# mousecpn/Boosting-R-CNN

Measured on AMD Instinct MI355X. Metric: images/sec (1333x800) Boosting R-CNN R50-PAFPN inference, higher is better.
Workload: dtype f32; 1 GPU; boosting_rcnn_r50_pafpn_1x_utdac.py inference (model(return_loss=False, rescale=True): device pass + result copy + bbox2result), batch 8 x 3x800x1344 per GPU, f32 MFMA conv stack, 1000 pre-NMS / 256 proposals per image, seeded synthetic weights; global_batch=8, parallelism=dp1

## Files before the change

### boosting-r-cnn_amd/csrc/misc.hip

```cpp
#include "common.h"

namespace {

__device__ __forceinline__ float4 ld4(const float* p) { return *reinterpret_cast<const float4*>(p); }
__device__ __forceinline__ void st4(float* p, float4 v) { *reinterpret_cast<float4*>(p) = v; }
__device__ __forceinline__ float4 ld4(const bf16_t* p) {
    const uint2 u = *reinterpret_cast<const uint2*>(p);
    return make_float4(__uint_as_float(u.x << 16), __uint_as_float(u.x & 0xffff0000u),
                       __uint_as_float(u.y << 16), __uint_as_float(u.y & 0xffff0000u));
}
__device__ __forceinline__ unsigned f2bf(float v) { return brcnn_f2b(v); }
__device__ __forceinline__ void st4(bf16_t* p, float4 v) {
    uint2 u;
    u.x = brcnn_pk2b(v.x, v.y);
    u.y = brcnn_pk2b(v.z, v.w);
    *reinterpret_cast<uint2*>(p) = u;
}
__device__ __forceinline__ float4 ld4(const f16_t* p) {
    const uint2 u = *reinterpret_cast<const uint2*>(p);
    return make_float4(brcnn_h2f((unsigned short)(u.x & 0xffffu)), brcnn_h2f((unsigned short)(u.x >> 16)),
                       brcnn_h2f((unsigned short)(u.y & 0xffffu)), brcnn_h2f((unsigned short)(u.y >> 16)));
}
__device__ __forceinline__ void st4(f16_t* p, float4 v) {
    uint2 u;
// ... 895 lines not shown
    } else {
        if (int st = gn_forward_16<f16_t>(x, gamma, beta, y, stats_ws, sg, batch, num_segments, channels, groups, eps,
                                          relu, chunks, rpb, total, nstat, s))
            return st;
    }
    BRCNN_LAUNCH_CHECK();
    return 0;
}


static int gn_setup(GnSegs& sg, long long& rows, int& max_hw, int batch, int num_segments, const int* hw_host) {
    sg = GnSegs{};
    sg.nseg = num_segments;
    rows = 0;
    max_hw = 0;
    for (int i = 0; i < num_segments; i++) {
        if (hw_host[i] <= 0) return BRCNN_EINVAL;
        sg.hw[i] = hw_host[i];
        sg.row0[i] = rows;
        rows += (long long)batch * hw_host[i];
        if (hw_host[i] > max_hw) max_hw = hw_host[i];
    }
    for (int i = num_segments; i <= BRCNN_MAX_LEVELS; i++) sg.row0[i] = rows;
    return 0;
}

static void gn_bwd_chunks(int max_hw, int* chunks, int* rpb) {
    int c = (max_hw + 255) / 256;
    if (c > 64) c = 64;
    *rpb = (max_hw + c - 1) / c;
    *chunks = (max_hw + *rpb - 1) / *rpb;
}

BRCNN_API size_t brcnn_groupnorm_nhwc_multi_backward_workspace_bytes(int batch, int num_segments, const int* hw_host,
                                                                    int channels, int groups) {
    if (batch <= 0 || num_segments <= 0 || num_segments > BRCNN_MAX_LEVELS || !hw_host || channels <= 0 || groups <= 0)
        return 0;
    int max_hw = 0;
    for (int i = 0; i < num_segments; i++) max_hw = hw_host[i] > max_hw ? hw_host[i] : max_hw;
    int chunks, rpb;
    gn_bwd_chunks(max_hw, &chunks, &rpb);
    return (size_t)batch * num_segments * groups * 2 * sizeof(double) +
           ((size_t)batch * num_segments * chunks + GN_PARAM_SLICES) * 2 * channels * sizeof(float);
}

BRCNN_API int brcnn_groupnorm_nhwc_multi_backward(const void* dy, const void* x, const void* stats,
// ... 238 lines not shown
```

### boosting-r-cnn_amd/csrc/policy.h

```cpp
#pragma once

namespace brcnn {

struct Policy {
    int use_dma = 1;
    int force_wm = 0, force_nt = 0;
    int no_fast = 0;
    int pp_f32_n128 = 1;
    int pp_f32_mode = 1;
    int f32_tile_sk = 1;
    int f32_tile_sk_per_cu = 0;

    int bf16_tile = 0;
    int bf16_il = 0;
    int sk_mode = 1;
    int sk_par = 0;
    int pp_mode = 1;
    int pp128_mode = 1;
    int pp128_min_k = 4096;
    int pp128_max_t88 = 128;
    int sk_spin_limit = 1 << 24;
    int sk_drop_publish = 0;
    int stream_mode = 1;

    int wgrad_bf16_tile = 0;
    int wgrad_slabs = 1;
    int wgrad_slot_pct = 75;
    int wgrad_slot_pct_big = 75;
    int wgrad_two_pass = 24;
    int wgrad_pp_mode = 1;
    int wgrad_pp_slot_pct = 75;
    int wgrad_pp_two_pass = 24;
    int wgrad_pp_fuse = 0;

// ... 6 lines not shown
};
extern Policy g_policy;

struct Counters {
    int f32_tile_sk_launches = 0;
    int f32_tile_sk_wgs = 0;
    int wgrad_pp_launches = 0;
    int pp_f32_launches = 0;
    int pp_f32_rows = 0;
    int pp_f32_cols = 0;
    int pp_bf16_launches = 0;
    int pp128_bf16_launches = 0;
    int stream1x1_launches = 0;
    int sk_chain_fills = 0;
    int sk_par_fills = 0;
    int sk_last_wgs = 0;
    int bf16_tile_launches = 0;
    int bf16_tile_rows = 0;
    int bf16_tile_cols = 0;
    int bf16_tile_waves = 0;
    int bf16_tile_stages = 0;
    int wgrad_bf16_tile_launches = 0;
    int wgrad_bf16_last_tile = 0;
    int roi_ordered_launches = 0;
    int roi_prepared_launches = 0;
    int roi_gather_chunked = 0;
    int roi_gather_last_ch = 0;
};
extern Counters g_counters;
inline void count(int& c) { c = (c + 1) & 0x7fffffff; }

}
```

### boosting-r-cnn_amd/csrc/policy.hip

```cpp
#include "common.h"
#include "policy.h"

__attribute__((require_constant_initialization)) brcnn::Policy brcnn::g_policy;
__attribute__((require_constant_initialization)) brcnn::Counters brcnn::g_counters;
using brcnn::g_counters, brcnn::g_policy;

BRCNN_API int brcnn_conv_set_tile(int wm, int nt) {
    if (wm == -1) { g_policy.use_dma = nt; return 0; }
    if (wm == -3) { if (nt < 0 || nt > 2) return BRCNN_EINVAL; g_policy.pp_f32_n128 = nt; return 0; }
    if (wm == -4) { if (nt != 0 && nt != 1) return BRCNN_EINVAL; g_policy.no_fast = nt; return 0; }
    if (wm == -5) { if (nt < 0 || nt > 2) return BRCNN_EINVAL; g_policy.f32_tile_sk = nt; return 0; }
    if (wm == -7) { if (nt < 0 || nt > 8) return BRCNN_EINVAL; g_policy.f32_tile_sk_per_cu = nt; return 0; }
    if (wm == -6) return nt == 0 ? g_counters.f32_tile_sk_launches : nt == 1 ? g_counters.f32_tile_sk_wgs : BRCNN_EINVAL;
    if (wm == -9) {
        int* const c[] = {&g_counters.pp_f32_launches, &g_counters.pp_f32_rows, &g_counters.pp_f32_cols, &g_counters.pp_bf16_launches,
                          &g_counters.pp128_bf16_launches, &g_counters.stream1x1_launches, &g_counters.sk_chain_fills,
                          &g_counters.sk_par_fills, &g_counters.sk_last_wgs, &g_counters.bf16_tile_launches, &g_counters.bf16_tile_rows,
                          &g_counters.bf16_tile_cols, &g_counters.bf16_tile_waves, &g_counters.bf16_tile_stages,
                          &g_counters.wgrad_bf16_tile_launches, &g_counters.wgrad_bf16_last_tile};
        const int count = (int)(sizeof(c) / sizeof(c[0]));
        if (nt < -1 || nt >= count) return BRCNN_EINVAL;
        if (nt == -1) { for (int* q : c) *q = 0; return 0; }
        const int n = *c[nt];
        *c[nt] = 0;
        return n;
    }
    if (wm == -2) { if (nt != 0 && nt != 1 && nt != 2 && nt != 128 && nt != 256) return BRCNN_EINVAL; g_policy.pp_f32_mode = nt; return 0; }
    if ((wm != 0 && wm != 1 && wm != 2 && wm != 4) || nt < 0 || nt > 2) return BRCNN_EINVAL;
    g_policy.force_wm = wm;
    g_policy.force_nt = nt;
    return 0;
}

BRCNN_API int brcnn_conv_set_tile_bf16(int mtnt) {
    if (mtnt == -1 || mtnt == -2) { g_policy.bf16_il = (mtnt == -1); return 0; }
    if (mtnt <= -3 && mtnt >= -5) { g_policy.sk_mode = -3 - mtnt; return 0; }
    if (mtnt <= -8 && mtnt >= -10) { g_policy.sk_par = -8 - mtnt; return 0; }
    if (mtnt == -6 || mtnt == -7) { g_policy.pp_mode = mtnt == -7; return 0; }
    if (mtnt == -18 || mtnt == -19) { g_policy.pp128_mode = mtnt == -19; return 0; }
    if (mtnt <= -1000 && mtnt > -2000) { g_policy.pp128_min_k = -1000 - mtnt; return 0; }
    if (mtnt <= -2000 && mtnt > -3000) { g_policy.pp128_max_t88 = -2000 - mtnt; return 0; }
    if (mtnt <= -15 && mtnt >= -17) { g_policy.stream_mode = -15 - mtnt; return 0; }
    if (mtnt == -11 || mtnt == -12) { g_policy.sk_drop_publish = mtnt == -11; g_policy.sk_spin_limit = mtnt == -11 ? 256 : 1 << 24; return 0; }
    const int ok[] = {0, 11, 21, 22, 42, 82, 81, 164, 342, 382, 3164, 322, 482, 381, 2244, 2144, 8844, 8842};
    bool found = false;
    for (int v : ok) found |= (v == mtnt);
    if (!found) return BRCNN_EINVAL;
// ... 84 lines not shown
```

### boosting-r-cnn_amd/dense_heads.py

```python
import copy

import torch
import torch.distributed as dist
import torch.nn as nn

from . import ops
from .blocks import (ConvModule, PackedCache, Scale, bias_init_with_prob, pack_weight, to_nhwc)
from .postprocess import batched_nms_images
from .core import (anchor_inside_flags, bbox_overlaps, images_to_levels, multi_apply, unmap)
from .registry import (HEADS, build_anchor_generator, build_assigner, build_bbox_coder,
                       build_loss, build_sampler)

EPS = 1e-12


def cat_rows(feats):
    from .autograd import cat_rows as _cr
    return _cr(list(feats))


def reduce_mean(tensor):
    if not (dist.is_available() and dist.is_initialized()):
        return tensor
    tensor = tensor.clone()
# ... 91 lines not shown
                sampling_result)


@HEADS.register_module()
class ATSSRPNHead(AnchorHead):
    def __init__(self, in_channels, num_classes=1, stacked_convs=4, conv_cfg=None, gamma=1,
                 atss=False, bridge=False, last_conv='norm', aug_reg_loss=None,
                 norm_cfg=dict(type='GN', num_groups=32, requires_grad=True),
                 loss_centerness=dict(type='CrossEntropyLoss', use_sigmoid=True, loss_weight=0.5),
                 init_cfg=None, num_convs=1, **kwargs):
        assert not atss, 'atss=True (ATSSAssigner targets) is outside the shipped boosting configs'
        assert not bridge and last_conv == 'norm', 'bridge / dcn / aspp variants are out of scope'
        self.stacked_convs, self.conv_cfg, self.norm_cfg = stacked_convs, conv_cfg, norm_cfg
        self.last_conv = last_conv
        super().__init__(num_classes, in_channels, init_cfg=init_cfg, **kwargs)
        self.loss_centerness = build_loss(loss_centerness)
        self.gamma, self.atss, self.bridge = gamma, atss, bridge
        self.with_aug_loss = aug_reg_loss is not None
        if self.with_aug_loss:
            self.aug_loss = build_loss(aug_reg_loss)
        self._head_caches = [PackedCache() for _ in range(8)]
        self._tower_caches = [PackedCache() for _ in range(stacked_convs)]
        self._fused_head_cache = PackedCache()
        self._base_anchor_cache = {}
        self.init_weights()

    def _init_layers(self):
        self.rpn_convs = nn.ModuleList()
        for i in range(self.stacked_convs):
            chn = self.in_channels if i == 0 else self.feat_channels
            self.rpn_convs.append(ConvModule(chn, self.feat_channels, 3, stride=1, padding=1,
                                             conv_cfg=self.conv_cfg, norm_cfg=self.norm_cfg))
        self.rpn_cls = nn.Conv2d(self.feat_channels, self.num_anchors * self.cls_out_channels, 3,
                                 padding=1)
        self.rpn_reg = nn.Conv2d(self.feat_channels, self.num_anchors * 4, 3, padding=1)
        self.rpn_iou = nn.Conv2d(self.feat_channels, self.num_anchors * 1, 3, padding=1)
        self.scales = nn.ModuleList([Scale(1.0) for _ in self.anchor_generator.strides])

    def init_weights(self):
        for m in self.modules():
            if isinstance(m, nn.Conv2d):
                nn.init.normal_(m.weight, 0, 0.01)
                if m.bias is not None:
                    nn.init.constant_(m.bias, 0)
        nn.init.constant_(self.rpn_cls.bias, bias_init_with_prob(0.01))

# ... 50 lines not shown
        for conv in self.rpn_convs:
            x = conv2d_nhwc_multi_autograd(x, conv.conv.weight, None, B, sizes, 1, conv.conv.padding[0])
            x = GroupNormNHWCFunction.apply(x, conv.norm.weight, conv.norm.bias, conv.norm.num_groups, B, sizes,
                                            conv.norm.eps, conv.with_activation)
        heads = (self.rpn_cls, self.rpn_reg, self.rpn_iou)
        y = conv2d_nhwc_multi_autograd(x, torch.cat([h.weight for h in heads], 0),
                                       torch.cat([h.bias for h in heads], 0), B, sizes, 1,
                                       self.rpn_cls.padding[0], out_f32=True).float()
        a, c = self.num_anchors, self.cls_out_channels
        cls, reg, iou, r0 = [], [], [], 0
        for lvl, (h, w) in enumerate(sizes):
            n = B * h * w
            t = y[r0:r0 + n].view(B, h, w, y.shape[1])
            cls.append(t[..., :a * c])
            reg.append(t[..., a * c:a * c + 4 * a] * self.scales[lvl].scale)
            iou.append(t[..., a * c + 4 * a:])
            r0 += n
        return cls, reg, iou

    def forward_fused(self, feats):
        B = feats[0].shape[0]
        sizes = [tuple(f.shape[1:3]) for f in feats]
        x = cat_rows(feats)
        for i, conv in enumerate(self.rpn_convs):
            assert isinstance(conv.norm, nn.GroupNorm) and conv.conv.bias is None
            w = self._tower_caches[i].get([conv.conv.weight],
                                          lambda c=conv: pack_weight(c.conv.weight).to(x.dtype))
            x, _ = ops.conv2d_nhwc_multi(x, w, B, sizes, None, None, None, False, 1, 1)
            x = ops.groupnorm_nhwc_multi(x, conv.norm.weight.detach(), conv.norm.bias.detach(),
                                         conv.norm.num_groups, B, sizes, conv.norm.eps,
                                         conv.with_activation)
        heads = (self.rpn_cls, self.rpn_reg, self.rpn_iou)

        def builder():
            return (torch.cat([pack_weight(h.weight) for h in heads], 0).to(x.dtype).contiguous(),
                    torch.cat([h.bias.detach().float() for h in heads], 0).contiguous())
        w, b = self._fused_head_cache.get([t for h in heads for t in (h.weight, h.bias)], builder)
        y, _ = ops.conv2d_nhwc_multi(x, w, B, sizes, None, b, None, False, 1, 1, out_f32=True)
        outs, r0 = [], 0
        for (h, wd) in sizes:
            n = B * h * wd
            outs.append(y[r0:r0 + n].view(B, h, wd, y.shape[1]))
            r0 += n
        return outs

    def split_fused(self, fused):
        a, c = self.num_anchors, self.cls_out_channels
        cls = [f[..., :a * c] for f in fused]
        reg = [f[..., a * c:a * c + 4 * a] for f in fused]
        iou = [f[..., a * c + 4 * a:] for f in fused]
        return cls, reg, iou

    def forward(self, feats, bridge=False):
        cls, reg, iou = self.forward_nhwc([to_nhwc(f) for f in feats])
# ... 406 lines not shown
```

### boosting-r-cnn_amd/detectors.py

```python
from collections import OrderedDict

import torch
import torch.distributed as dist
import torch.nn as nn

from .blocks import to_nchw_view, to_nhwc
from .core import bbox2result
from .profiling import stage_mark
from .registry import DETECTORS, build_backbone, build_head, build_neck

HOLD_RPN_WGRAD = __import__('os').environ.get('BRCNN_HOLD_RPN_WGRAD', '1')


class LazyLogVars(OrderedDict):

    def __init__(self, names, vals):
        super().__init__()
        self._names = list(names)
        self._pending = None
        if vals.is_cuda:
            self._host = torch.empty(vals.shape, dtype=vals.dtype).pin_memory()
            self._host.copy_(vals, non_blocking=True)
            self._pending = torch.cuda.Event()
            self._pending.record()
# ... 138 lines not shown
        if neck is not None:
            self.neck = build_neck(neck)
        if rpn_head is not None:
            rpn_train_cfg = train_cfg.rpn if train_cfg is not None else None
            rpn_head_ = rpn_head.copy()
            rpn_head_.update(train_cfg=rpn_train_cfg, test_cfg=test_cfg.rpn)
            self.rpn_head = build_head(rpn_head_)
        if roi_head is not None:
            rcnn_train_cfg = train_cfg.rcnn if train_cfg is not None else None
            roi_head = roi_head.copy()
            roi_head.update(train_cfg=rcnn_train_cfg)
            roi_head.update(test_cfg=test_cfg.rcnn)
            self.roi_head = build_head(roi_head)
        self.train_cfg, self.test_cfg = train_cfg, test_cfg
        self._rpn_scale_cache = None

    def set_compute_dtype(self, dtype):
        from . import blocks
        blocks.set_compute_dtype(dtype)
        return self

    def freeze_for_inference(self):
        self._rpn_scale_cache = [float(m.scale.detach().cpu()) for m in self.rpn_head.scales]
        return self

    def extract_feat_nhwc(self, img):
        tap = None
        if self.with_neck and torch.is_grad_enabled() and hasattr(self.neck, 'lateral_tap') and \
                getattr(self.backbone, 'supports_tap', False):
            self.neck.__dict__.pop('_pre_laterals', None)
            tap = self.neck.lateral_tap
        if hasattr(self.backbone, 'forward_from_nchw'):
            x = self.backbone.forward_from_nchw(img, tap) if tap is not None else self.backbone.forward_from_nchw(img)
        else:
            x = self.backbone.forward_nhwc(to_nhwc(img), tap) if tap is not None else self.backbone.forward_nhwc(to_nhwc(img))
        stage_mark('backbone')
        if self.with_neck:
            x = self.neck.forward_nhwc(x)
            stage_mark('neck')
        return x

    def extract_feat(self, img):
        return tuple(to_nchw_view(f) for f in self.extract_feat_nhwc(img))

    def _device_train_ok(self, img, gt_bboxes_ignore, proposals):
        return (img.is_cuda and self.with_rpn and proposals is None and gt_bboxes_ignore is None and
# ... 191 lines not shown
```

### boosting-r-cnn_amd/lib.py

```python
import ctypes
import os

_HERE = os.path.dirname(os.path.abspath(__file__))
LIB_PATH = os.environ.get('BRCNN_LIB_PATH') or os.path.join(_HERE, 'lib', 'libbrcnn_hip.so')
_lib = None

c_int, c_i64, c_f32, c_f64, c_ptr, c_size = (ctypes.c_int, ctypes.c_int64, ctypes.c_float,
                                             ctypes.c_double, ctypes.c_void_p, ctypes.c_size_t)

SIGNATURES = {
    'brcnn_version': (c_int, []),
    'brcnn_device_count': (c_int, []),
    'brcnn_roi_align_forward': (c_int, [c_ptr] * 5 + [c_int] * 7 + [c_f32] + [c_int] * 4 + [c_ptr]),
    'brcnn_roi_align_backward': (c_int, [c_ptr] * 3 + [c_int] * 7 + [c_f32] + [c_int] * 3 + [c_ptr]),
    'brcnn_roi_extract_forward': (c_int, [c_ptr] * 4 + [c_int] + [c_ptr] * 3 + [c_int] * 6 +
                                  [c_f32, c_int, c_ptr]),
    'brcnn_roi_extract_forward_ordered': (c_int, [c_ptr] * 4 + [c_int] + [c_ptr] * 3 + [c_int] * 6 +
                                          [c_f32, c_int, c_ptr, c_ptr]),
    'brcnn_roi_extract_prep_workspace_bytes': (c_size, [c_int]),
    'brcnn_roi_extract_order_min_rois': (c_int, []),
    'brcnn_roi_extract_forward_prepared': (c_int, [c_ptr] * 4 + [c_int] + [c_ptr] * 3 + [c_int] * 6 +
                                           [c_f32, c_int, c_ptr, c_ptr, c_size, c_ptr]),
    'brcnn_get_tuning': (c_int, [c_ptr]),
    'brcnn_set_tuning': (c_int, [c_ptr]),
# ... 1 lines not shown
                                   [c_f32, c_ptr]),
    'brcnn_roi_extract_backward_workspace_bytes': (c_size, [c_int]),
    'brcnn_roi_extract_backward_workspace_bytes_ex': (c_size, [c_int, c_int, c_int, c_int, c_ptr, c_ptr]),
    'brcnn_roi_extract_backward_gather': (c_int, [c_ptr] * 4 + [c_int] + [c_ptr] * 2 + [c_int] * 6 + [c_f32, c_ptr, c_size,
                                                                                                    c_int, c_ptr]),
    'brcnn_roi_extract_backward_gather_add': (c_int, [c_ptr] * 5 + [c_int] + [c_ptr] * 2 + [c_int] * 6 + [c_f32, c_ptr, c_size,
                                                                                                        c_int, c_ptr]),
    'brcnn_nms_workspace_bytes': (c_size, [c_i64, c_int, c_i64]),
    'brcnn_nms': (c_int, [c_ptr] * 4 + [c_int, c_i64, c_i64, c_f32, c_int, c_int, c_ptr, c_ptr,
                                        c_ptr, c_size, c_ptr]),
    'brcnn_softnms_workspace_bytes': (c_size, [c_i64, c_int]),
    'brcnn_softnms': (c_int, [c_ptr] * 4 + [c_int, c_i64, c_f32, c_f32, c_f32, c_int, c_int,
                                            c_ptr, c_ptr, c_ptr, c_ptr, c_size, c_ptr]),
    'brcnn_sigmoid_focal_loss_forward': (c_int, [c_ptr] * 4 + [c_i64, c_i64, c_f32, c_f32, c_ptr]),
    'brcnn_sigmoid_focal_loss_backward': (c_int, [c_ptr] * 4 + [c_i64, c_i64, c_f32, c_f32, c_ptr]),
    'brcnn_conv2d_nhwc': (c_int, [c_ptr] * 6 + [c_int] * 11 + [c_ptr]),
    'brcnn_conv_set_tile': (c_int, [c_int, c_int]),
    'brcnn_clock_probe': (c_int, [c_ptr, c_i64, c_ptr]),
    'brcnn_nms_prepare': (c_int, [c_ptr] * 9 + [c_int, c_int, c_ptr]),
    'brcnn_nms_collect': (c_int, [c_ptr] * 7 + [c_int, c_int, c_int, c_ptr]),
    'brcnn_conv2d_nhwc_scatter2': (c_int, [c_ptr] * 3 + [c_int] * 14 + [c_ptr]),
    'brcnn_conv2d_nhwc_multi': (c_int, [c_ptr] * 6 + [c_int, c_int, c_ptr, c_ptr] + [c_int] * 8 +
                                [c_ptr]),
    'brcnn_conv2d_dgrad_nhwc_multi': (c_int, [c_ptr] * 3 + [c_int, c_int] + [c_ptr] * 4 + [c_int] * 7 +
                                      [c_ptr]),
    'brcnn_conv2d_wgrad_nhwc_multi': (c_int, [c_ptr] * 3 + [c_int, c_int] + [c_ptr] * 2 + [c_int] * 7 +
                                      [c_ptr]),
    'brcnn_wgrad_defer_begin': (c_int, [c_ptr, c_ptr, c_size, c_int]),
    'brcnn_wgrad_defer_flush': (c_int, [c_ptr]),
    'brcnn_wgrad_defer_pending': (c_int, [c_ptr]),
    'brcnn_wgrad_defer_stats': (c_int, [c_ptr, c_ptr, c_ptr]),
    'brcnn_stem_workspace_bytes': (c_size, [c_int, c_int, c_int]),
    'brcnn_stem7x7s2_nchw': (c_int, [c_ptr] * 6 + [c_int] * 6 + [c_ptr]),
    'brcnn_stem7x7s2_pool_nchw': (c_int, [c_ptr] * 5 + [c_int] * 5 + [c_ptr]),
    'brcnn_bottleneck_tail_f32': (c_int, [c_ptr] * 9 + [c_int] * 3 + [c_ptr]),
    'brcnn_bottleneck_tail_16': (c_int, [c_ptr] * 9 + [c_int] * 4 + [c_ptr]),
    'brcnn_conv_set_tile_bf16': (c_int, [c_int]),
    'brcnn_conv_workspace_bytes': (c_size, []),
    'brcnn_conv_set_workspace': (c_int, [c_ptr, c_ptr, c_size]),
    'brcnn_conv_handover_status': (c_int, []),
    'brcnn_maxpool3x3s2_nhwc': (c_int, [c_ptr] * 2 + [c_int] * 5 + [c_ptr]),
    'brcnn_maxpool3x3s2_nhwc_backward': (c_int, [c_ptr] * 4 + [c_int] * 5 + [c_ptr]),
    'brcnn_groupnorm_nhwc': (c_int, [c_ptr] * 5 + [c_int] * 4 + [c_f32, c_int, c_int, c_ptr]),
    'brcnn_groupnorm_nhwc_multi': (c_int, [c_ptr] * 5 + [c_int, c_int, c_ptr, c_int, c_int, c_f32,
                                                          c_int, c_int, c_ptr]),
    'brcnn_groupnorm_nhwc_multi_backward_workspace_bytes': (c_size, [c_int, c_int, c_ptr, c_int, c_int]),
# ... 186 lines not shown
```

### boosting-r-cnn_amd/ops.py

```python
import math

import numpy as np
import torch
import torch.nn as nn
from torch.autograd import Function
from torch.autograd.function import once_differentiable

from . import lib as _L

LAYOUT_NCHW, LAYOUT_NHWC = 0, 1
DT_F32, DT_BF16, DT_BF16_OUT_F32, DT_F16, DT_F16_OUT_F32 = 0, 1, 2, 3, 4


def _dt(t):
    if t.dtype == torch.float32:
        return DT_F32
    if t.dtype == torch.bfloat16:
        return DT_BF16
    if t.dtype == torch.float16:
        return DT_F16
    raise _L.BrcnnHipError(f'unsupported activation dtype {t.dtype} (fp32, bf16 or fp16)')


def _out_f32(dt):
# ... 560 lines not shown
    st = _L.load().brcnn_conv2d_nhwc_multi(_ptr(x_cat), _ptr(w), _ptr(scale), _ptr(shift),
                                           _ptr(residual), _ptr(y), batch, L, hs, ws, cin, cout, kh,
                                           kw, int(stride), int(pad), int(bool(relu)), dt,
                                           _conv_stream())
    _L.check(st, 'brcnn_conv2d_nhwc_multi')
    return y, out_sizes


def groupnorm_nhwc_multi(x_cat, gamma, beta, groups, batch, sizes, eps=1e-5, relu=False, return_stats=False):
    import ctypes
    _require_gpu(x_cat, gamma, beta)
    L = len(sizes)
    c = x_cat.shape[1]
    y = torch.empty_like(x_cat)
    ws = torch.empty((batch * L * groups * 2,), dtype=torch.float64, device=x_cat.device)
    hw = (ctypes.c_int * L)(*[h * w for h, w in sizes])
    st = _L.load().brcnn_groupnorm_nhwc_multi(_ptr(x_cat), _ptr(gamma), _ptr(beta), _ptr(y), _ptr(ws),
                                              batch, L, hw, c, int(groups), float(eps),
                                              int(bool(relu)), _dt(x_cat), _stream())
    _L.check(st, 'brcnn_groupnorm_nhwc_multi')
    return (y, ws) if return_stats else y


def groupnorm_nhwc_multi_backward(dy, x_cat, stats, gamma, beta, groups, batch, sizes, relu):
    import ctypes
    _require_gpu(dy, x_cat, stats, gamma, beta)
    assert dy.shape == x_cat.shape and dy.dtype == x_cat.dtype and dy.is_contiguous() and x_cat.is_contiguous()
    L = len(sizes)
    c = x_cat.shape[1]
    hw = (ctypes.c_int * L)(*[h * w for h, w in sizes])
    lib = _L.load()
    nbytes = lib.brcnn_groupnorm_nhwc_multi_backward_workspace_bytes(batch, L, hw, c, int(groups))
    ws = torch.empty((nbytes + 7) // 8, dtype=torch.float64, device=x_cat.device)
    dx = torch.empty_like(x_cat)
    dgamma = torch.empty(c, dtype=torch.float32, device=x_cat.device)
    dbeta = torch.empty(c, dtype=torch.float32, device=x_cat.device)
    st = lib.brcnn_groupnorm_nhwc_multi_backward(_ptr(dy), _ptr(x_cat), _ptr(stats), _ptr(gamma), _ptr(beta),
                                                 _ptr(dx), _ptr(dgamma), _ptr(dbeta), _ptr(ws), nbytes, batch, L, hw,
                                                 c, int(groups), int(bool(relu)), _dt(x_cat), _stream())
    _L.check(st, 'brcnn_groupnorm_nhwc_multi_backward')
    return dx, dgamma, dbeta


def pack_stem_weight(w, dtype=torch.float32):
    cout = w.shape[0]
    p = torch.zeros((cout, 8, 8, 4), dtype=torch.float32, device=w.device)
# ... 618 lines not shown
```

### include/brcnn_hip.h

```cpp
#ifndef BRCNN_HIP_H
#define BRCNN_HIP_H

#include <stddef.h>
#include <stdint.h>

#ifdef __cplusplus
extern "C" {
#endif

#define BRCNN_LAYOUT_NCHW 0
#define BRCNN_LAYOUT_NHWC 1

#define BRCNN_DT_F32 0
#define BRCNN_DT_BF16 1
#define BRCNN_DT_BF16_OUT_F32 2
#define BRCNN_DT_F16 3
#define BRCNN_DT_F16_OUT_F32 4

#define BRCNN_MAX_LEVELS 8
#define BRCNN_MAX_IMAGES 64

int brcnn_version(void);

int brcnn_clock_probe(int64_t *out2, int64_t wall_ticks_100mhz, void *stream);
// ... 118 lines not shown
                      int cout, int kh, int kw, int stride, int pad, int relu, int dtype,
                      void *stream);

int brcnn_conv2d_nhwc_scatter2(const void *x, const void *w, void *y, int batch, int height, int width,
                               int cin, int cout, int kh, int kw, int pad, int out_height,
                               int out_width, int ph, int pw, int origin, int dtype, void *stream);

size_t brcnn_conv_workspace_bytes(void);
int brcnn_conv_set_workspace(void *stream, void *workspace, size_t bytes);

#define BRCNN_EHANDOVER (-62)
int brcnn_conv_handover_status(void);

int brcnn_conv_set_tile(int wm, int nt);

int brcnn_conv_set_tile_bf16(int mtnt);

int brcnn_conv2d_nhwc_multi(const void *x, const void *w, const float *scale, const float *shift,
                            const void *residual, void *y, int batch, int num_segments,
                            const int *heights_host, const int *widths_host, int cin, int cout,
                            int kh, int kw, int stride, int pad, int relu, int dtype,
                            void *stream);

int brcnn_conv2d_nhwc_grouped(const void *x, const void *w_tiles, const float *scale,
                              const float *shift, const void *residual, void *y, int batch,
                              int height, int width, int cin, int cout, int kh, int kw, int stride,
                              int pad, int window, int relu, int dtype, void *stream);
int brcnn_conv2d_dgrad_nhwc_grouped(const void *dy, const void *w_t_tiles, void *dx, int batch,
                                    int in_height, int in_width, int out_height, int out_width, int cin,
                                    int cout, int kh, int kw, int stride, int pad, int window, int dtype,
                                    void *stream);
int brcnn_conv2d_wgrad_nhwc_grouped(const void *x, const void *dy, void *dw_tiles, int batch, int height,
                                    int width, int cin, int cout, int kh, int kw, int stride, int pad,
                                    int window, int dtype, void *stream);

int brcnn_conv2d_dgrad_nhwc_multi(const void *dy, const void *w_t, void *dx, int batch,
                                  int num_segments, const int *in_heights_host,
                                  const int *in_widths_host, const int *out_heights_host,
                                  const int *out_widths_host, int cin, int cout, int kh, int kw,
                                  int stride, int pad, int dtype, void *stream);
int brcnn_conv2d_wgrad_nhwc_multi(const void *x, const void *dy, void *dw, int batch,
                                  int num_segments, const int *heights_host,
                                  const int *widths_host, int cin, int cout, int kh, int kw,
                                  int stride, int pad, int dtype, void *stream);
int brcnn_wgrad_defer_begin(void *stream, void *arena, size_t bytes, int max_items);
int brcnn_wgrad_defer_flush(void *stream);
// ... 12 lines not shown
                              void *y, int batch, int height, int width, int cout, int dtype, void *stream);

int brcnn_bottleneck_tail_f32(const float *x, const float *w2, const float *scale2, const float *shift2, const float *w3,
                              const float *scale3, const float *shift3, const float *identity, float *y, int batch,
                              int height, int width, void *stream);
int brcnn_bottleneck_tail_16(const void *x, const void *w2, const float *scale2, const float *shift2, const void *w3,
                             const float *scale3, const float *shift3, const void *identity, void *y, int batch,
                             int height, int width, int dtype, void *stream);

int brcnn_maxpool3x3s2_nhwc(const void *x, void *y, int batch, int height, int width,
                            int channels, int dtype, void *stream);
int brcnn_maxpool3x3s2_nhwc_backward(const void *x, const void *y, const void *dy, void *dx, int batch,
                                     int height, int width, int channels, int dtype, void *stream);

int brcnn_groupnorm_nhwc(const void *x, const float *gamma, const float *beta, void *y,
                         void *stats_ws ,
                         int batch, int hw, int channels, int groups, float eps, int relu,
                         int dtype, void *stream);

int brcnn_groupnorm_nhwc_multi(const void *x, const float *gamma, const float *beta, void *y,
                               void *stats_ws ,
                               int batch, int num_segments, const int *hw_host, int channels,
                               int groups, float eps, int relu, int dtype, void *stream);

size_t brcnn_groupnorm_nhwc_multi_backward_workspace_bytes(int batch, int num_segments, const int *hw_host,
                                                           int channels, int groups);
int brcnn_groupnorm_nhwc_multi_backward(const void *dy, const void *x, const void *stats, const float *gamma,
                                        const float *beta, void *dx, float *dgamma, float *dbeta,
                                        void *workspace, size_t workspace_bytes, int batch, int num_segments,
                                        const int *hw_host, int channels, int groups, int relu, int dtype,
                                        void *stream);

int brcnn_bn_act_forward(const void *z, const float *scale, const float *shift, const void *residual,
                         void *out, int64_t rows, int channels, int relu, int dtype, void *stream);
size_t brcnn_bn_act_backward_workspace_bytes(int64_t rows, int channels, int dtype);
int brcnn_bn_act_backward(const void *dout, const void *out, const void *z, const float *scale,
                          void *dz, void *dres, float *dscale, float *dshift, void *workspace,
                          size_t workspace_bytes, int64_t rows, int channels, int relu, int dtype,
                          void *stream);

int brcnn_conv2d_bn_act_nhwc_multi(const void *x, const void *w, const float *gamma, const float *beta,
                                   const float *mean, const float *var, float eps, const void *residual,
                                   void *z_out, void *y, int batch, int num_segments,
                                   const int *heights_host, const int *widths_host, int cin, int cout,
                                   int kh, int kw, int stride, int pad, int relu, int dtype, void *stream);

// ... 229 lines not shown
```

Baseline: 340.4 images/sec.

## Add Winograd F(2x2,3x3) f32 conv path for RPN tower with fused GroupNorm input

Adds a Winograd F(2,3) path for the 3x3 stride-1 RPN tower convolutions. The filter is transformed once and cached at freeze time, the input transform applies the previous layer's GroupNorm and ReLU, and 16 MFMA GEMMs write output tiles straight to NHWC. This cuts the multiply count of the 3x3 convs and avoids a separate GroupNorm apply pass between tower layers. The cost is extra workspace traffic for the transformed input and some f32 numerical drift. Whether it runs by default depends on a policy flag queried through winograd_enabled.

```diff
diff --git a/boosting-r-cnn_amd/csrc/conv_winograd_f32.hip b/boosting-r-cnn_amd/csrc/conv_winograd_f32.hip
--- /dev/null
+++ b/boosting-r-cnn_amd/csrc/conv_winograd_f32.hip
@@ -0,0 +1,377 @@
+#include "conv_common.h"
+#include "policy.h"
+
+namespace {
+using namespace brcnn_conv;
+
+typedef __attribute__((address_space(3))) void* lds_ptr_t;
+
+struct WinoSegs {
+    int nseg, batch;
+    int H[BRCNN_MAX_LEVELS], W[BRCNN_MAX_LEVELS], TH[BRCNN_MAX_LEVELS], TW[BRCNN_MAX_LEVELS];
+    int t0[BRCNN_MAX_LEVELS + 1];
+    int r0[BRCNN_MAX_LEVELS + 1];
+};
+
+struct WinoTile { int seg, n, h, w; };
+__device__ __forceinline__ WinoTile wino_tile(const WinoSegs& sg, int t) {
+    int s = 0;
+#pragma unroll
+    for (int i = 1; i < BRCNN_MAX_LEVELS; i++)
+        if (i < sg.nseg && t >= sg.t0[i]) s = i;
+    const int l = t - sg.t0[s];
+    const int per = sg.TH[s] * sg.TW[s];
+    const int n = l / per, rem = l - n * per;
+    const int th = rem / sg.TW[s];
+    return {s, n, 2 * th, 2 * (rem - th * sg.TW[s])};
+}
+
+__global__ __launch_bounds__(256) void wino_filter_kernel(const float* __restrict__ w, float* __restrict__ u, int Cout, int Cin) {
+    const int idx = blockIdx.x * 256 + threadIdx.x;
+    if (idx >= Cout * Cin) return;
+    const int co = idx / Cin, ci = idx - co * Cin;
+    float g[3][3], t[4][3];
+#pragma unroll
+    for (int a = 0; a < 3; a++)
+#pragma unroll
+        for (int b = 0; b < 3; b++) g[a][b] = w[((size_t)(co * 3 + a) * 3 + b) * Cin + ci];
+#pragma unroll
+    for (int b = 0; b < 3; b++) {
+        t[0][b] = g[0][b];
+        t[1][b] = 0.5f * (g[0][b] + g[1][b] + g[2][b]);
+        t[2][b] = 0.5f * (g[0][b] - g[1][b] + g[2][b]);
+        t[3][b] = g[2][b];
+    }
+#pragma unroll
+    for (int a = 0; a < 4; a++) {
+        const float o[4] = {t[a][0], 0.5f * (t[a][0] + t[a][1] + t[a][2]), 0.5f * (t[a][0] - t[a][1] + t[a][2]), t[a][2]};
+#pragma unroll
+        for (int b = 0; b < 4; b++) u[((size_t)(a * 4 + b) * Cout + co) * Cin + ci] = o[b];
+    }
+}
+
+__global__ __launch_bounds__(256) void wino_input_kernel(const float* __restrict__ x, float* __restrict__ v, WinoSegs sg,
+                                                        int tile0, int nt, int C, const double* __restrict__ stats,
+                                                        const float* __restrict__ gamma, const float* __restrict__ beta,
+                                                        int G, int relu_in) {
+    const int cq = C >> 2;
+    const unsigned idx = blockIdx.x * 256u + threadIdx.x;
+    if (idx >= (unsigned)nt * (unsigned)cq) return;
+    const int tl = (int)(idx / (unsigned)cq), c0 = ((int)idx - tl * cq) * 4;
+    const WinoTile t = wino_tile(sg, tile0 + tl);
+    const int H = sg.H[t.seg], W = sg.W[t.seg];
+    const float* xs = x + ((size_t)sg.r0[t.seg] + (size_t)t.n * H * W) * C + c0;
+    float mean[4], rstd[4], gm[4], bt[4];
+    if (stats) {
+        const int cpg = C / G;
+#pragma unroll
+        for (int e = 0; e < 4; e++) {
+            const int c = c0 + e;
+            const float2 mr = reinterpret_cast<const float2*>(stats + ((size_t)(t.seg * sg.batch + t.n) * G + c / cpg) * 2)[0];
+            mean[e] = mr.x; rstd[e] = mr.y; gm[e] = gamma[c]; bt[e] = beta[c];
+        }
+    }
+    float d[4][4][4];
+#pragma unroll
+    for (int a = 0; a < 4; a++)
+#pragma unroll
+        for (int b = 0; b < 4; b++) {
+            const int h = t.h - 1 + a, w = t.w - 1 + b;
+            const bool ok = (unsigned)h < (unsigned)H && (unsigned)w < (unsigned)W;
+            float4 q = make_float4(0.f, 0.f, 0.f, 0.f);
+            if (ok) q = *reinterpret_cast<const float4*>(xs + ((size_t)h * W + w) * C);
+            float in[4] = {q.x, q.y, q.z, q.w};
+            if (stats) {
+#pragma unroll
+                for (int e = 0; e < 4; e++) {
+                    const float o = (in[e] - mean[e]) * rstd[e] * gm[e] + bt[e];
+                    in[e] = ok ? (relu_in ? fmaxf(o, 0.f) : o) : 0.f;
+                }
+            }
+#pragma unroll
+            for (int e = 0; e < 4; e++) d[a][b][e] = in[e];
+        }
+    float* vs = v + (size_t)tl * C + c0;
+    const size_t xi_stride = (size_t)nt * C;
+#pragma unroll
+    for (int e = 0; e < 4; e++) {
+        float r[4][4];
+#pragma unroll
+        for (int b = 0; b < 4; b++) {
+            r[0][b] = d[0][b][e] - d[2][b][e];
+            r[1][b] = d[1][b][e] + d[2][b][e];
+            r[2][b] = d[2][b][e] - d[1][b][e];
+            r[3][b] = d[1][b][e] - d[3][b][e];
+        }
+#pragma unroll
+        for (int a = 0; a < 4; a++) {
+            d[a][0][e] = r[a][0] - r[a][2];
+            d[a][1][e] = r[a][1] + r[a][2];
+            d[a][2][e] = r[a][2] - r[a][1];
+            d[a][3][e] = r[a][1] - r[a][3];
+        }
+    }
+#pragma unroll
+    for (int a = 0; a < 4; a++)
+#pragma unroll
+        for (int b = 0; b < 4; b++)
+            *reinterpret_cast<float4*>(vs + (size_t)(a * 4 + b) * xi_stride) = make_float4(d[a][b][0], d[a][b][1], d[a][b][2], d[a][b][3]);
+}
+
+struct WinoGemmParams {
+    const float* v;
+    const float* u;
+    const float* scale;
+    const float* shift;
+    float* y;
+    unsigned v_bytes, u_bytes;
+    int tile0, nt, Cin, Cout, relu;
+    int tiles_m, tiles_n;
+    WinoSegs sg;
+};
+
+constexpr int WBM = 64, WBN = 128;
+
+__device__ __forceinline__ constexpr int wino_at(int a, int i) { return a == 0 ? (i < 3 ? 1 : 0) : (i == 0 ? 0 : (i == 1 ? 1 : -1)); }
+
+__global__ __launch_bounds__(256, 2) void wino_gemm_kernel(WinoGemmParams p) {
+    __shared__ __attribute__((aligned(16))) float smem[2 * WBM * 32 + 2 * WBN * 32];
+    float* As = smem;
+    float* Bs = smem + 2 * WBM * 32;
+    const int tid = threadIdx.x;
+    const int lane = tid & 63;
+    const int wave = __builtin_amdgcn_readfirstlane(tid >> 6);
+    const int wm = wave >> 1, wn = wave & 1;
+    const int li = lane & 31, lh = lane >> 5;
+
+    const int tile = xcd_remap(blockIdx.x, p.tiles_m * p.tiles_n);
+    const int tile_m = tile / p.tiles_n, tile_n = tile - tile_m * p.tiles_n;
+    const int m0 = tile_m * WBM, n0 = tile_n * WBN;
+
+    const __amdgpu_buffer_rsrc_t rsrc_v = __builtin_amdgcn_make_buffer_rsrc((void*)p.v, 0, (int)p.v_bytes, 0x00020000);
+    const __amdgpu_buffer_rsrc_t rsrc_u = __builtin_amdgcn_make_buffer_rsrc((void*)p.u, 0, (int)p.u_bytes, 0x00020000);
+
+    constexpr int AG = WBM / 8 / 4, BG = WBN / 8 / 4;
+    const int rg = lane >> 3, pc = lane & 7;
+    int a_off[AG], b_off[BG];
+#pragma unroll
+    for (int j = 0; j < AG; j++) {
+        const int r = (wave * AG + j) * 8 + rg;
+        const int t = m0 + r;
+        a_off[j] = t < p.nt ? (t * p.Cin + (pc ^ ((r >> 1) & 7)) * 4) * 4 : -1;
+    }
+#pragma unroll
+    for (int j = 0; j < BG; j++) {
+        const int r = (wave * BG + j) * 8 + rg;
+        const int co = n0 + r;
+        b_off[j] = co < p.Cout ? (co * p.Cin + (pc ^ ((r >> 1) & 7)) * 4) * 4 : -1;
+    }
+    const int nk = p.Cin / 32;
+    const int a_xi = p.nt * p.Cin * 4, b_xi = p.Cout * p.Cin * 4;
+    int s_xi = 0, s_kc = 0;
+    auto dma_step = [&](int buf) {
+        const int ao = s_xi * a_xi + s_kc * 128, bo = s_xi * b_xi + s_kc * 128;
+        if (++s_kc == nk) { s_kc = 0; s_xi++; }
+#pragma unroll
+        for (int j = 0; j < AG; j++) {
+            float* dst = As + buf * WBM * 32 + (wave * AG + j) * 8 * 32;
+            __builtin_amdgcn_raw_ptr_buffer_load_lds(rsrc_v, (lds_ptr_t)dst, 16, a_off[j] >= 0 ? a_off[j] + ao : OOB, 0, 0, 0);
+        }
+#pragma unroll
+        for (int j = 0; j < BG; j++) {
+            float* dst = Bs + buf * WBN * 32 + (wave * BG + j) * 8 * 32;
+            __builtin_amdgcn_raw_ptr_buffer_load_lds(rsrc_u, (lds_ptr_t)dst, 16, b_off[j] >= 0 ? b_off[j] + bo : OOB, 0, 0, 0);
+        }
+    };
+
+    const int sw = (li >> 1) & 7;
+    unsigned chb[4];
+#pragma unroll
+    for (int kk = 0; kk < 4; kk++) chb[kk] = (unsigned)(((2 * kk + lh) ^ sw) * 16);
+    const unsigned a_lane = (unsigned)(size_t)(lds_ptr_t)(As + (wm * 32 + li) * 32);
+    const unsigned b_lane = (unsigned)(size_t)(lds_ptr_t)(Bs + (wn * 64 + li) * 32);
+    f32x4 av[2], bv[2][2];
+    auto frag_read = [&](int slot, unsigned a_addr, unsigned b_addr) {
+        asm volatile("ds_read_b128 %0, %1" : "=v"(av[slot]) : "v"(a_addr) : "memory");
+        asm volatile("ds_read_b128 %0, %1" : "=v"(bv[slot][0]) : "v"(b_addr) : "memory");
+        asm volatile("ds_read_b128 %0, %1 offset:4096" : "=v"(bv[slot][1]) : "v"(b_addr) : "memory");
+    };
+    auto frag_wait = [&](int slot) {
+        asm volatile("s_waitcnt lgkmcnt(0)" : "+v"(av[slot]), "+v"(bv[slot][0]), "+v"(bv[slot][1]) :: "memory");
+    };
+
+    f32x16 yacc[4][2], tmp[2];
+#pragma unroll
+    for (int q = 0; q < 4; q++)
+#pragma unroll
+        for (int b = 0; b < 2; b++)
+#pragma unroll
+            for (int r = 0; r < 16; r++) yacc[q][b][r] = 0.f;
+
+    dma_step(0);
+    asm volatile("s_waitcnt vmcnt(0)" ::: "memory");
+    __syncthreads();
+    int cur = 0;
+    for (int xi = 0; xi < 16; xi++) {
+#pragma unroll
+        for (int b = 0; b < 2; b++)
+#pragma unroll
+            for (int r = 0; r < 16; r++) tmp[b][r] = 0.f;
+        for (int kc = 0; kc < nk; kc++) {
+            const unsigned a_cur = a_lane + cur * (WBM * 32 * 4);
+            const unsigned b_cur = b_lane + cur * (WBN * 32 * 4);
+            frag_read(0, a_cur + chb[0], b_cur + chb[0]);
+            if (xi < 15 || kc + 1 < nk) dma_step(cur ^ 1);
+            frag_wait(0);
+#pragma unroll
+            for (int kk = 0; kk < 4; kk++) {
+                const int sl = kk & 1;
+                if (kk + 1 < 4) frag_read(sl ^ 1, a_cur + chb[kk + 1], b_cur + chb[kk + 1]);
+#pragma unroll
+                for (int e = 0; e < 4; e++)
+#pragma unroll
+                    for (int b = 0; b < 2; b++)
+                        tmp[b] = __builtin_amdgcn_mfma_f32_32x32x2f32(av[sl][e], bv[sl][b][e], tmp[b], 0, 0, 0);
+                if (kk + 1 < 4) frag_wait(sl ^ 1);
+            }
+            asm volatile("s_waitcnt vmcnt(0)" ::: "memory");
+            __syncthreads();
+            cur ^= 1;
+        }
+        const int i = xi >> 2, j = xi & 3;
+#pragma unroll
+        for (int a = 0; a < 2; a++)
+#pragma unroll
+            for (int bq = 0; bq < 2; bq++) {
+                const float c = (float)(wino_at(a, i) * wino_at(bq, j));
+#pragma unroll
+                for (int b = 0; b < 2; b++)
+#pragma unroll
+                    for (int r = 0; r < 16; r++) yacc[a * 2 + bq][b][r] = __builtin_fmaf(c, tmp[b][r], yacc[a * 2 + bq][b][r]);
+            }
+    }
+
+    float* slab = smem + wave * 1024;
+    const int vrow = lane >> 3, vcol = (lane & 7) * 4;
+    long long prow[4];
+    int pw[4], pflag[4];
+#pragma unroll
+    for (int it = 0; it < 4; it++) {
+        const int tl = m0 + wm * 32 + it * 8 + vrow;
+        prow[it] = -1; pw[it] = 0; pflag[it] = 0;
+        if (tl < p.nt) {
+            const WinoTile t = wino_tile(p.sg, p.tile0 + tl);
+            const int H = p.sg.H[t.seg], W = p.sg.W[t.seg];
+            prow[it] = ((long long)p.sg.r0[t.seg] + ((long long)t.n * H + t.h) * W + t.w) * p.Cout;
+            pw[it] = W;
+            pflag[it] = (t.w + 1 < W ? 1 : 0) | (t.h + 1 < H ? 2 : 0);
+        }
+    }
+    float* __restrict__ yout = p.y;
+#pragma unroll
+    for (int b = 0; b < 2; b++) {
+        const int co = n0 + wn * 64 + b * 32 + li;
+        const bool cok = co < p.Cout;
+        const float sc = (p.scale && cok) ? p.scale[co] : 1.f;
+        const float sh = (p.shift && cok) ? p.shift[co] : 0.f;
+        const int cv = n0 + wn * 64 + b * 32 + vcol;
+#pragma unroll
+        for (int q = 0; q < 4; q++) {
+#pragma unroll
+            for (int r = 0; r < 16; r++) {
+                float o = yacc[q][b][r];
+                if (p.scale) o = o * sc;
+                slab[((r & 3) + 8 * (r >> 2) + 4 * lh) * 32 + li] = o + sh;
+            }
+            __builtin_amdgcn_s_waitcnt(0xc07f);
+            __builtin_amdgcn_wave_barrier();
+#pragma unroll
+            for (int it = 0; it < 4; it++) {
+                float4 o = *reinterpret_cast<const float4*>(slab + (it * 8 + vrow) * 32 + vcol);
+                if (p.relu) { o.x = fmaxf(o.x, 0.f); o.y = fmaxf(o.y, 0.f); o.z = fmaxf(o.z, 0.f); o.w = fmaxf(o.w, 0.f); }
+                const bool in_map = ((q & 1) == 0 || (pflag[it] & 1)) && ((q & 2) == 0 || (pflag[it] & 2));
+                if (prow[it] >= 0 && in_map && cv < p.Cout)
+                    *reinterpret_cast<float4*>(yout + prow[it] + (long long)((q >> 1) * pw[it] + (q & 1)) * p.Cout + cv) = o;
+            }
+            __builtin_amdgcn_s_waitcnt(0xc07f);
+            __builtin_amdgcn_wave_barrier();
+        }
+    }
+}
+
+int wino_segs(WinoSegs& sg, int batch, int num_segments, const int* heights_host, const int* widths_host) {
+    if (batch <= 0 || num_segments <= 0 || num_segments > BRCNN_MAX_LEVELS || !heights_host || !widths_host) return BRCNN_EINVAL;
+    sg = {};
+    sg.nseg = num_segments;
+    sg.batch = batch;
+    long long tiles = 0, rows = 0;
+    for (int s = 0; s < num_segments; s++) {
+        const int H = heights_host[s], W = widths_host[s];
+        if (H <= 0 || W <= 0 || H >= 4096 || W >= 4096) return BRCNN_EINVAL;
+        sg.H[s] = H; sg.W[s] = W; sg.TH[s] = (H + 1) / 2; sg.TW[s] = (W + 1) / 2;
+        sg.t0[s] = (int)tiles; sg.r0[s] = (int)rows;
+        tiles += (long long)batch * sg.TH[s] * sg.TW[s];
+        rows += (long long)batch * H * W;
+        if (rows > 0x7fffffffLL / 4) return BRCNN_EINVAL;
+    }
+    for (int s = num_segments; s <= BRCNN_MAX_LEVELS; s++) { sg.t0[s] = (int)tiles; sg.r0[s] = (int)rows; }
+    return 0;
+}
+
+}
+
+BRCNN_API size_t brcnn_conv3x3_winograd_f32_multi_workspace_bytes(int batch, int num_segments, const int* heights_host,
+                                                                  const int* widths_host, int cin) {
+    WinoSegs sg;
+    if (cin <= 0 || wino_segs(sg, batch, num_segments, heights_host, widths_host)) return 0;
+    return (size_t)16 * (size_t)sg.t0[num_segments] * (size_t)cin * sizeof(float);
+}
+
+BRCNN_API int brcnn_winograd_filter_f32(const void* w, void* u, int cout, int cin, int kh, int kw, int dtype, void* stream) {
+    if (!w || !u || dtype != BRCNN_DT_F32 || kh != 3 || kw != 3 || cin <= 0 || cout <= 0 || (cin % 32) || (cout % 64) ||
+        (long long)cout * cin * 64 >= 0x7fffffffLL)
+        return BRCNN_EINVAL;
+    hipLaunchKernelGGL(wino_filter_kernel, dim3((cout * cin + 255) / 256), dim3(256), 0, (hipStream_t)stream, (const float*)w,
+                       (float*)u, cout, cin);
+    BRCNN_LAUNCH_CHECK();
+    return 0;
+}
+
+BRCNN_API int brcnn_conv3x3_winograd_f32_multi(const void* x, const void* u, const void* gn_stats, const float* gamma,
+                                               const float* beta, int groups, int relu_in, const float* scale,
+                                               const float* shift, int relu, void* y, void* workspace, size_t workspace_bytes,
+                                               int batch, int num_segments, const int* heights_host, const int* widths_host,
+                                               int cin, int cout, int kh, int kw, int stride, int pad, int dtype, void* stream) {
+    if (!x || !u || !y || !workspace || dtype != BRCNN_DT_F32 || kh != 3 || kw != 3 || stride != 1 || pad != 1 || cin <= 0 ||
+        cout <= 0 || (cin % 32) || (cout % 64) || (long long)cout * cin * 64 >= 0x7fffffffLL)
+        return BRCNN_EINVAL;
+    if (gn_stats && (!gamma || !beta || groups <= 0 || cin % groups)) return BRCNN_EINVAL;
+    WinoGemmParams p = {};
+    if (wino_segs(p.sg, batch, num_segments, heights_host, widths_host)) return BRCNN_EINVAL;
+    const int tiles = p.sg.t0[num_segments];
+    if ((long long)p.sg.r0[num_segments] * (cin > cout ? cin : cout) * 4 >= 0x7fffffffLL) return BRCNN_EINVAL;
+    if (workspace_bytes < (size_t)16 * tiles * cin * sizeof(float)) return BRCNN_EINVAL;
+    int chunks = brcnn::g_policy.f32_winograd_chunks;
+    while ((long long)16 * ((tiles + chunks - 1) / chunks + WBM) * cin * 4 >= 0x7fffffffLL) chunks *= 2;
+    const int per = ((tiles + chunks - 1) / chunks + WBM - 1) / WBM * WBM;
+    hipStream_t s = (hipStream_t)stream;
+    p.v = (const float*)workspace; p.u = (const float*)u; p.scale = scale; p.shift = shift; p.y = (float*)y;
+    p.u_bytes = (unsigned)((long long)cout * cin * 64);
+    p.Cin = cin; p.Cout = cout; p.relu = relu;
+    p.tiles_n = (cout + WBN - 1) / WBN;
+    for (int t0 = 0; t0 < tiles; t0 += per) {
+        const int nt = tiles - t0 < per ? tiles - t0 : per;
+        const long long th = (long long)nt * (cin >> 2);
+        hipLaunchKernelGGL(wino_input_kernel, dim3((unsigned)((th + 255) / 256)), dim3(256), 0, s, (const float*)x, (float*)workspace,
+                           p.sg, t0, nt, cin, (const double*)gn_stats, gamma, beta, groups, relu_in);
+        BRCNN_LAUNCH_CHECK();
+        p.tile0 = t0; p.nt = nt;
+        p.v_bytes = (unsigned)((long long)16 * nt * cin * 4);
+        p.tiles_m = (nt + WBM - 1) / WBM;
+        hipLaunchKernelGGL(wino_gemm_kernel, dim3(p.tiles_m * p.tiles_n), dim3(256), 0, s, p);
+        BRCNN_LAUNCH_CHECK();
+    }
+    brcnn::count(brcnn::g_counters.f32_winograd_launches);
+    brcnn::g_counters.f32_winograd_tiles = tiles;
+    return 0;
+}
diff --git a/boosting-r-cnn_amd/csrc/misc.hip b/boosting-r-cnn_amd/csrc/misc.hip
--- a/boosting-r-cnn_amd/csrc/misc.hip
+++ b/boosting-r-cnn_amd/csrc/misc.hip
@@ -941,6 +941,32 @@
         if (hw_host[i] > max_hw) max_hw = hw_host[i];
     }
     for (int i = num_segments; i <= BRCNN_MAX_LEVELS; i++) sg.row0[i] = rows;
+    return 0;
+}
+
+BRCNN_API int brcnn_groupnorm_nhwc_multi_stats(const void* x, void* stats_ws, int batch, int num_segments, const int* hw_host,
+                                               int channels, int groups, float eps, int dtype, void* stream) {
+    if (!x || !stats_ws || batch <= 0 || num_segments <= 0 || num_segments > BRCNN_MAX_LEVELS || !hw_host || channels <= 0 ||
+        channels > 256 || groups <= 0 || channels % groups || (channels & 3) || dtype != BRCNN_DT_F32)
+        return BRCNN_EINVAL;
+    GnSegs sg;
+    long long rows;
+    int max_hw;
+    if (gn_setup(sg, rows, max_hw, batch, num_segments, hw_host)) return BRCNN_EINVAL;
+    if (rows * channels >= 0x7fffffffLL) return BRCNN_EINVAL;
+    hipStream_t s = (hipStream_t)stream;
+    BRCNN_HIP_CHECK(hipMemsetAsync(stats_ws, 0, (size_t)batch * num_segments * groups * 2 * sizeof(double), s));
+    int chunks = (max_hw + 255) / 256;
+    if (chunks > 512) chunks = 512;
+    const int rpb = (max_hw + chunks - 1) / chunks;
+    chunks = (max_hw + rpb - 1) / rpb;
+    const int nstat = num_segments * batch * groups;
+    hipLaunchKernelGGL((gn_stats_kernel<float, 4>), dim3(chunks, batch * num_segments), dim3(256), 0, s, (const float*)x,
+                       (double*)stats_ws, sg, batch, channels, groups, rpb);
+    BRCNN_LAUNCH_CHECK();
+    hipLaunchKernelGGL(gn_finalize_kernel, dim3((nstat + 255) / 256), dim3(256), 0, s, (double*)stats_ws, sg, batch, channels,
+                       groups, eps);
+    BRCNN_LAUNCH_CHECK();
     return 0;
 }
 
diff --git a/boosting-r-cnn_amd/csrc/policy.h b/boosting-r-cnn_amd/csrc/policy.h
--- a/boosting-r-cnn_amd/csrc/policy.h
+++ b/boosting-r-cnn_amd/csrc/policy.h
@@ -10,6 +10,8 @@
     int pp_f32_mode = 1;
     int f32_tile_sk = 1;
     int f32_tile_sk_per_cu = 0;
+    int f32_winograd = 1;
+    int f32_winograd_chunks = 1;
 
     int bf16_tile = 0;
     int bf16_il = 0;
@@ -62,6 +64,8 @@
     int bf16_tile_stages = 0;
     int wgrad_bf16_tile_launches = 0;
     int wgrad_bf16_last_tile = 0;
+    int f32_winograd_launches = 0;
+    int f32_winograd_tiles = 0;
     int roi_ordered_launches = 0;
     int roi_prepared_launches = 0;
     int roi_gather_chunked = 0;
diff --git a/boosting-r-cnn_amd/csrc/policy.hip b/boosting-r-cnn_amd/csrc/policy.hip
--- a/boosting-r-cnn_amd/csrc/policy.hip
+++ b/boosting-r-cnn_amd/csrc/policy.hip
@@ -20,9 +20,26 @@
                           &g_counters.wgrad_bf16_tile_launches, &g_counters.wgrad_bf16_last_tile};
         const int count = (int)(sizeof(c) / sizeof(c[0]));
         if (nt < -1 || nt >= count) return BRCNN_EINVAL;
-        if (nt == -1) { for (int* q : c) *q = 0; return 0; }
+        if (nt == -1) {
+            for (int* q : c) *q = 0;
+            g_counters.f32_winograd_launches = g_counters.f32_winograd_tiles = 0;
+            return 0;
+        }
         const int n = *c[nt];
         *c[nt] = 0;
+        return n;
+    }
+    if (wm == -11) {
+        if (nt == 0 || nt == 1) { g_policy.f32_winograd = nt; return 0; }
+        if (nt == 2) return g_policy.f32_winograd;
+        if (nt >= 11 && nt <= 18) { g_policy.f32_winograd_chunks = nt - 10; return 0; }
+        return BRCNN_EINVAL;
+    }
+    if (wm == -12) {
+        if (nt != 0 && nt != 1) return BRCNN_EINVAL;
+        int& c = nt == 0 ? g_counters.f32_winograd_launches : g_counters.f32_winograd_tiles;
+        const int n = c;
+        c = 0;
         return n;
     }
     if (wm == -2) { if (nt != 0 && nt != 1 && nt != 2 && nt != 128 && nt != 256) return BRCNN_EINVAL; g_policy.pp_f32_mode = nt; return 0; }
diff --git a/boosting-r-cnn_amd/dense_heads.py b/boosting-r-cnn_amd/dense_heads.py
--- a/boosting-r-cnn_amd/dense_heads.py
+++ b/boosting-r-cnn_amd/dense_heads.py
@@ -137,6 +137,8 @@
         self._head_caches = [PackedCache() for _ in range(8)]
         self._tower_caches = [PackedCache() for _ in range(stacked_convs)]
         self._fused_head_cache = PackedCache()
+        self._wino_caches = [PackedCache() for _ in range(stacked_convs)]
+        self._wino_prepared = False
         self._base_anchor_cache = {}
         self.init_weights()
 
@@ -233,6 +235,9 @@
         B = feats[0].shape[0]
         sizes = [tuple(f.shape[1:3]) for f in feats]
         x = cat_rows(feats)
+        if self._wino_prepared and x.dtype == torch.float32 and self._winograd_ok() and ops.winograd_enabled():
+            x = self._tower_winograd(x, B, sizes)
+            return self._fused_heads(x, B, sizes)
         for i, conv in enumerate(self.rpn_convs):
             assert isinstance(conv.norm, nn.GroupNorm) and conv.conv.bias is None
             w = self._tower_caches[i].get([conv.conv.weight],
@@ -241,6 +246,37 @@
             x = ops.groupnorm_nhwc_multi(x, conv.norm.weight.detach(), conv.norm.bias.detach(),
                                          conv.norm.num_groups, B, sizes, conv.norm.eps,
                                          conv.with_activation)
+        return self._fused_heads(x, B, sizes)
+
+    def prepare_winograd(self):
+        self._wino_prepared = True
+        if self._winograd_ok() and self.rpn_convs[0].conv.weight.is_cuda and ops.winograd_enabled():
+            for i, conv in enumerate(self.rpn_convs):
+                self._wino_filter(i, conv)
+        return self
+
+    def _winograd_ok(self):
+        return all(isinstance(c.norm, nn.GroupNorm) and c.conv.bias is None and c.conv.groups == 1 and
+                   c.conv.kernel_size == (3, 3) and c.conv.stride == (1, 1) and c.conv.padding == (1, 1) and
+                   c.conv.dilation == (1, 1) and c.conv.in_channels % 32 == 0 and c.conv.out_channels % 64 == 0 and
+                   c.conv.out_channels <= 256 for c in self.rpn_convs)
+
+    def _wino_filter(self, i, conv):
+        return self._wino_caches[i].get([conv.conv.weight], lambda: ops.winograd_filter(pack_weight(conv.conv.weight)))
+
+    def _tower_winograd(self, x, B, sizes):
+        ws = ops.winograd_workspace(B, sizes, max(c.conv.in_channels for c in self.rpn_convs), x.device)
+        gn, last = None, len(self.rpn_convs) - 1
+        for i, conv in enumerate(self.rpn_convs):
+            x = ops.conv3x3_winograd_multi(x, self._wino_filter(i, conv), B, sizes, gn=gn, workspace=ws)
+            norm = conv.norm
+            if i == last:
+                return ops.groupnorm_nhwc_multi(x, norm.weight.detach(), norm.bias.detach(), norm.num_groups, B, sizes,
+                                                norm.eps, conv.with_activation)
+            gn = (ops.groupnorm_stats_multi(x, norm.num_groups, B, sizes, norm.eps), norm.weight.detach(),
+                  norm.bias.detach(), norm.num_groups, conv.with_activation)
+
+    def _fused_heads(self, x, B, sizes):
         heads = (self.rpn_cls, self.rpn_reg, self.rpn_iou)
 
         def builder():
diff --git a/boosting-r-cnn_amd/detectors.py b/boosting-r-cnn_amd/detectors.py
--- a/boosting-r-cnn_amd/detectors.py
+++ b/boosting-r-cnn_amd/detectors.py
@@ -184,6 +184,8 @@
 
     def freeze_for_inference(self):
         self._rpn_scale_cache = [float(m.scale.detach().cpu()) for m in self.rpn_head.scales]
+        if hasattr(self.rpn_head, 'prepare_winograd'):
+            self.rpn_head.prepare_winograd()
         return self
 
     def extract_feat_nhwc(self, img):
diff --git a/boosting-r-cnn_amd/lib.py b/boosting-r-cnn_amd/lib.py
--- a/boosting-r-cnn_amd/lib.py
+++ b/boosting-r-cnn_amd/lib.py
@@ -47,6 +47,11 @@
     'brcnn_conv2d_nhwc_scatter2': (c_int, [c_ptr] * 3 + [c_int] * 14 + [c_ptr]),
     'brcnn_conv2d_nhwc_multi': (c_int, [c_ptr] * 6 + [c_int, c_int, c_ptr, c_ptr] + [c_int] * 8 +
                                 [c_ptr]),
+    'brcnn_winograd_filter_f32': (c_int, [c_ptr, c_ptr] + [c_int] * 5 + [c_ptr]),
+    'brcnn_conv3x3_winograd_f32_multi_workspace_bytes': (c_size, [c_int, c_int, c_ptr, c_ptr, c_int]),
+    'brcnn_conv3x3_winograd_f32_multi': (c_int, [c_ptr] * 5 + [c_int, c_int, c_ptr, c_ptr, c_int, c_ptr, c_ptr, c_size,
+                                                 c_int, c_int, c_ptr, c_ptr] + [c_int] * 7 + [c_ptr]),
+    'brcnn_groupnorm_nhwc_multi_stats': (c_int, [c_ptr, c_ptr, c_int, c_int, c_ptr, c_int, c_int, c_f32, c_int, c_ptr]),
     'brcnn_conv2d_dgrad_nhwc_multi': (c_int, [c_ptr] * 3 + [c_int, c_int] + [c_ptr] * 4 + [c_int] * 7 +
                                       [c_ptr]),
     'brcnn_conv2d_wgrad_nhwc_multi': (c_int, [c_ptr] * 3 + [c_int, c_int] + [c_ptr] * 2 + [c_int] * 7 +
diff --git a/boosting-r-cnn_amd/ops.py b/boosting-r-cnn_amd/ops.py
--- a/boosting-r-cnn_amd/ops.py
+++ b/boosting-r-cnn_amd/ops.py
@@ -606,6 +606,70 @@
     return (y, ws) if return_stats else y
 
 
+def groupnorm_stats_multi(x_cat, groups, batch, sizes, eps=1e-5):
+    import ctypes
+    _require_gpu(x_cat)
+    L = len(sizes)
+    ws = torch.empty((batch * L * groups * 2,), dtype=torch.float64, device=x_cat.device)
+    hw = (ctypes.c_int * L)(*[h * w for h, w in sizes])
+    st = _L.load().brcnn_groupnorm_nhwc_multi_stats(_ptr(x_cat), _ptr(ws), batch, L, hw, x_cat.shape[1], int(groups),
+                                                    float(eps), _dt(x_cat), _stream())
+    _L.check(st, 'brcnn_groupnorm_nhwc_multi_stats')
+    return ws
+
+
+def winograd_enabled():
+    return _L.load().brcnn_conv_set_tile(-11, 2) == 1
+
+
+def winograd_filter(w):
+    _require_gpu(w)
+    assert w.dim() == 4 and w.is_contiguous()
+    cout, kh, kw, cin = w.shape
+    u = torch.empty((16, cout, cin), dtype=torch.float32, device=w.device)
+    st = _L.load().brcnn_winograd_filter_f32(_ptr(w), _ptr(u), cout, cin, kh, kw, _dt(w), _stream())
+    _L.check(st, 'brcnn_winograd_filter_f32')
+    return u
+
+
+_WINO_WS = {}
+
+
+def winograd_workspace(batch, sizes, cin, device):
+    import ctypes
+    L = len(sizes)
+    hs = (ctypes.c_int * L)(*[h for h, _ in sizes])
+    ws = (ctypes.c_int * L)(*[ww for _, ww in sizes])
+    nbytes = _L.load().brcnn_conv3x3_winograd_f32_multi_workspace_bytes(batch, L, hs, ws, cin)
+    key = (str(torch.device(device)), _stream())
+    t = _WINO_WS.get(key)
+    if t is None or t.numel() < nbytes:
+        t = _WINO_WS[key] = _ws(nbytes, device)
+    return t
+
+
+def conv3x3_winograd_multi(x_cat, u, batch, sizes, gn=None, scale=None, shift=None, relu=False, workspace=None,
+                           kernel=3, stride=1, pad=1):
+    import ctypes
+    stats, gamma, beta, groups, relu_in = gn if gn is not None else (None, None, None, 0, False)
+    _require_gpu(x_cat, u, scale, shift, stats, gamma, beta)
+    assert x_cat.dim() == 2 and x_cat.is_contiguous() and u.is_contiguous() and u.dim() == 3 and u.shape[0] == 16
+    _, cout, cin = u.shape
+    assert x_cat.shape[1] == cin and x_cat.shape[0] == sum(batch * h * ww for h, ww in sizes)
+    if workspace is None:
+        workspace = winograd_workspace(batch, sizes, cin, x_cat.device)
+    y = _alloc_out((x_cat.shape[0], cout), torch.float32, x_cat.device)
+    L = len(sizes)
+    hs = (ctypes.c_int * L)(*[h for h, _ in sizes])
+    ws = (ctypes.c_int * L)(*[ww for _, ww in sizes])
+    st = _L.load().brcnn_conv3x3_winograd_f32_multi(
+        _ptr(x_cat), _ptr(u), _ptr(stats), _ptr(gamma), _ptr(beta), int(groups), int(bool(relu_in)), _ptr(scale), _ptr(shift),
+        int(bool(relu)), _ptr(y), _ptr(workspace), workspace.numel() * workspace.element_size(), batch, L, hs, ws, cin, cout,
+        int(kernel), int(kernel), int(stride), int(pad), _dt(x_cat), _stream())
+    _L.check(st, 'brcnn_conv3x3_winograd_f32_multi')
+    return y
+
+
 def groupnorm_nhwc_multi_backward(dy, x_cat, stats, gamma, beta, groups, batch, sizes, relu):
     import ctypes
     _require_gpu(dy, x_cat, stats, gamma, beta)
diff --git a/include/brcnn_hip.h b/include/brcnn_hip.h
--- a/include/brcnn_hip.h
+++ b/include/brcnn_hip.h
@@ -164,6 +164,15 @@
                             int kh, int kw, int stride, int pad, int relu, int dtype,
                             void *stream);
 
+int brcnn_winograd_filter_f32(const void *w, void *u, int cout, int cin, int kh, int kw, int dtype, void *stream);
+size_t brcnn_conv3x3_winograd_f32_multi_workspace_bytes(int batch, int num_segments, const int *heights_host,
+                                                        const int *widths_host, int cin);
+int brcnn_conv3x3_winograd_f32_multi(const void *x, const void *u, const void *gn_stats, const float *gamma,
+                                     const float *beta, int groups, int relu_in, const float *scale,
+                                     const float *shift, int relu, void *y, void *workspace, size_t workspace_bytes,
+                                     int batch, int num_segments, const int *heights_host, const int *widths_host,
+                                     int cin, int cout, int kh, int kw, int stride, int pad, int dtype, void *stream);
+
 int brcnn_conv2d_nhwc_grouped(const void *x, const void *w_tiles, const float *scale,
                               const float *shift, const void *residual, void *y, int batch,
                               int height, int width, int cin, int cout, int kh, int kw, int stride,
@@ -222,6 +231,8 @@
                                void *stats_ws ,
                                int batch, int num_segments, const int *hw_host, int channels,
                                int groups, float eps, int relu, int dtype, void *stream);
+int brcnn_groupnorm_nhwc_multi_stats(const void *x, void *stats_ws, int batch, int num_segments, const int *hw_host,
+                                     int channels, int groups, float eps, int dtype, void *stream);
 
 size_t brcnn_groupnorm_nhwc_multi_backward_workspace_bytes(int batch, int num_segments, const int *hw_host,
                                                            int channels, int groups);
```

New measurement: 378.3 images/sec, median of 6. 11.1% higher.
